# huangeddie/GymGo

Hardware: AMD Instinct MI355X
Metric: env steps/sec across batched games, 19x19 uniform-random rollouts (higher is better)
Workload: dtype u8; 1 GPU; 19x19, 65536 parallel games, uniform-random rollouts with auto-reset; one bench step = one launch of 256 plies for every game; board=19, games=65536, games_per_gpu=65536, env_steps_per_bench_step=16777216, burn_in_steps=1, desync_plies=640

## Files before the change

### gymgo_amd/csrc/gg_r5.hip

```cpp
#include <hip/hip_runtime.h>
#include <stdint.h>

#include "gg_common.h"
#include "gg_v2.h"
#include "gg_v4.h"
#include "gg_v5.h"
#include "gg_ws.h"

namespace gg {

void launch_rollout5(int io, int N, uint8_t *st, uint64_t *rng, int32_t *last_actions, int64_t *steps_done, int64_t B, uint32_t inv,
                     int plies, int auto_reset, int nb, int grid, hipStream_t s, uint32_t *ws) {
#define GG_R5(R)                                                                                                                  \
  do {                                                                                                                            \
    if (io == 0) k_rollout5<R, 0><<<grid, kWave, 0, s>>>(st, rng, last_actions, steps_done, B, inv, plies, auto_reset, nb, ws);   \
    else k_rollout5<R, 2><<<grid, kWave, 0, s>>>(st, rng, last_actions, steps_done, B, inv, plies, auto_reset, nb, nullptr);      \
  } while (0)
  if (N == 19) GG_R5(19);
  else if (N == 13) GG_R5(13);
  else GG_R5(9);
#undef GG_R5
}

void launch_rollout5_policy(int N, uint8_t *st, uint64_t *rng, int32_t *last_actions, int64_t *steps_done, int64_t B, uint32_t inv,
                            int plies, int auto_reset, int nb, int grid, hipStream_t s) {
  if (N == 19) k_rollout5_pol<19, 2><<<grid, kWave, 0, s>>>(st, rng, last_actions, steps_done, B, inv, plies, auto_reset, nb, nullptr);
  else if (N == 13) k_rollout5_pol<13, 2><<<grid, kWave, 0, s>>>(st, rng, last_actions, steps_done, B, inv, plies, auto_reset, nb, nullptr);
  else k_rollout5_pol<9, 2><<<grid, kWave, 0, s>>>(st, rng, last_actions, steps_done, B, inv, plies, auto_reset, nb, nullptr);
}

}

#ifdef GG_AB_SWEEPS
extern "C" int32_t gg_ab_sweeps_read_r5(unsigned long long *out2) {
  if (hipDeviceSynchronize() != hipSuccess) return 1;
  if (hipMemcpyFromSymbol(out2, HIP_SYMBOL(gg::gg_sweeps), 16) != hipSuccess) return 2;
  unsigned long long z[2] = {0, 0};
  return hipMemcpyToSymbol(HIP_SYMBOL(gg::gg_sweeps), z, 16) == hipSuccess ? 0 : 3;
}
#endif

#ifdef GG_AB_PROF
GG_PROF_READ(gg_ab_prof_read_r5)
#endif

#ifdef GG_AB_P3
extern "C" int32_t gg_ab_p3_read_r5(unsigned long long *out10) {
  if (hipDeviceSynchronize() != hipSuccess) return 1;
  if (hipMemcpyFromSymbol(out10, HIP_SYMBOL(gg::gg_p3), 80) != hipSuccess) return 2;
  unsigned long long z[10] = {0, 0, 0, 0, 0, 0, 0, 0, 0, 0};
  return hipMemcpyToSymbol(HIP_SYMBOL(gg::gg_p3), z, 80) == hipSuccess ? 0 : 3;
}
#endif

#ifdef GG_AB_WS
extern "C" int32_t gg_ab_ws_read_r5(unsigned long long *out2) {
  if (hipDeviceSynchronize() != hipSuccess) return 1;
  if (hipMemcpyFromSymbol(out2, HIP_SYMBOL(gg::gg_wsc), 16) != hipSuccess) return 2;
  unsigned long long z[2] = {0, 0};
  return hipMemcpyToSymbol(HIP_SYMBOL(gg::gg_wsc), z, 16) == hipSuccess ? 0 : 3;
}
#endif

#ifdef GG_AB_LOADSPLIT
extern "C" int32_t gg_ab_load_split_read_r5(unsigned long long *out4) {
  if (hipDeviceSynchronize() != hipSuccess) return 1;
  if (hipMemcpyFromSymbol(out4, HIP_SYMBOL(gg::gg_lsplit), 32) != hipSuccess) return 2;
  unsigned long long z[4] = {0, 0, 0, 0};
  return hipMemcpyToSymbol(HIP_SYMBOL(gg::gg_lsplit), z, 32) == hipSuccess ? 0 : 3;
}
#endif

#if defined(GG_AB_P3) || defined(GG_AB_LIVE)
extern "C" int32_t gg_ab_live_bad_r5(unsigned long long *out1) {
  if (hipDeviceSynchronize() != hipSuccess) return 1;
  return hipMemcpyFromSymbol(out1, HIP_SYMBOL(gg::gg_live_bad), 8) == hipSuccess ? 0 : 2;
}
#endif
```

### gymgo_amd/csrc/gg_v5.h

```cpp
#pragma once
#include "gg_v4.h"

namespace gg {

constexpr int kNB5 = 32;
constexpr int kJobCap = 128;

template <int R>
struct Lds5 {
  static constexpr int RS = R == 13 ? 20 : Cfg<R>::kRowStride;
  static constexpr int RPL = (R + 1) / 2;
  static_assert(2 * RPL <= RS, "a pair's rows must fit the row stride");
  static constexpr int kPad = 4;
  static constexpr int kState = kPad;
  static constexpr int kMeta = kState + 2 * kNB5 * RS;
  static constexpr int kFair = kMeta + 5 * kNB5;
  static constexpr int kTmp = kFair + 16;
  static constexpr int kUnion = kTmp + 4 * RS;
  static constexpr int kZero = kJobCap, kDump = kJobCap + 1;
  static constexpr int kCls = kUnion;
  static constexpr int kJob = kCls + kJobCap + 4;
  static constexpr int kG = kJob + kJobCap + 4;
  static constexpr int kSc = kG + 2 * kNB5 * RS;
  static constexpr int kLoopEnd = kSc + kWave * RS;
  static constexpr int kV2 = kUnion;
  static constexpr int kIoEnd = kV2 + (Lds2<R>::kRegion0 > 768 ? Lds2<R>::kRegion0 : 768);
  static constexpr int kDmaWords = (((kNB5 * (5 * R + 1) * 4 + 12 + 15) / 16 + kWave - 1) / kWave) * 256;
  static constexpr int kDmaEnd = kUnion + kDmaWords;
  static constexpr int kGrpBits = kUnion;
  static constexpr int kGrpWords = ((15 + kNB5 * 6 * R * R + 31) / 32 + 4) & ~3;
  static constexpr int kGrpLut = kGrpBits + kGrpWords;
  static constexpr int kGrpEnd = kGrpLut + 512;
  static constexpr int kMax2(int a, int b) { return a > b ? a : b; }
  static constexpr int kTotal = kMax2(kMax2(kLoopEnd, kIoEnd), kMax2(kDmaEnd, kGrpEnd));
  static_assert(kTotal * 4 <= 20480, "two waves per SIMD: 20 KB of LDS per wave");
  static_assert(kUnion % 4 == 0 && kG % 4 == 0 && kSc % 4 == 0, "16-byte alignment of the flood blocks");
  static_assert(3 * kNB5 * RS <= kLoopEnd - kUnion, "parked tracked rows fit the loop area");
};

__device__ __forceinline__ uint32_t mbcnt64(uint64_t m) {
  return __builtin_amdgcn_mbcnt_hi((uint32_t)(m >> 32), __builtin_amdgcn_mbcnt_lo((uint32_t)m, 0u));
}
constexpr int QP_L0 = 0xA0;

__device__ __forceinline__ void kth_set_bit10(const uint32_t (&v)[10], const uint32_t (&p)[10], uint32_t tt, int &rr, uint32_t &pos) {
  uint32_t ntt = ~tt;
  const uint32_t g5 = (uint32_t)((int32_t)(p[4] + ntt) >> 31);
  uint32_t a[5], t[4];
#pragma unroll
  for (int i = 0; i < 5; ++i) a[i] = B3(g5, v[5 + i], v[i], T_SEL);
#pragma unroll
  for (int i = 0; i < 4; ++i) t[i] = B3(g5, p[5 + i], p[i], T_SEL);
  uint32_t base = g5 & p[4], row = g5 & 5u;
  const uint32_t g2 = (uint32_t)((int32_t)(t[1] + ntt) >> 31);
  const uint32_t b0 = B3(g2, a[2], a[0], T_SEL), b1 = B3(g2, a[3], a[1], T_SEL), u0 = B3(g2, t[2], t[0], T_SEL);
  base = B3(g2, t[1], base, T_SEL);
  row = B3(g2, 2u, row, T_ANDOR);
  const uint32_t g1 = (uint32_t)((int32_t)(u0 + ntt) >> 31);
  uint32_t vr = B3(g1, b1, b0, T_SEL);
  base = B3(g1, u0, base, T_SEL);
  row -= g1;
  const uint32_t g1b = B3(g2, g1, (uint32_t)((int32_t)(t[3] + ntt) >> 31), TA & TB & TC);
  vr = B3(g1b, a[4], vr, T_SEL);
  base = B3(g1b, t[3], base, T_SEL);
  row -= g1b;
  ntt += base;
  uint32_t ps = 0;
#pragma unroll
  for (int sh = 16; sh >= 1; sh >>= 1) {
    const uint32_t e = (uint32_t)__popc((vr >> ps) & ((1u << sh) - 1u)) + ntt;
    const uint32_t ge = (uint32_t)((int32_t)e >> 31);
    ntt = B3(ge, e, ntt, T_SEL);
    ps = B3((uint32_t)sh, ge, ps, T_ANDOR);
  }
  rr = (int)row;
  pos = ps;
}

template <int R, bool WEAK>
__device__ __forceinline__ void flood_jobs(const uint32_t (&m)[R], const uint32_t (&mrev)[R], uint32_t (&f)[R], uint32_t (&res)[R],
                                           bool need, const uint32_t (&mm)[R], uint32_t &open) {
  int sweeps = 0;
#pragma unroll 1
  for (int it = 0; it < R * R; ++it) {
#pragma unroll
    for (int r = 0; r < R; ++r) FLOOD_VISIT(r, r - 1, (r & 1) != 0);
    if (it > 0) {
      uint32_t op = 0, opw = 0, pend = 0, above = 0;
#pragma unroll
      for (int r = R - 1; r >= 0; --r) {
        const uint32_t g = ((r + 1) & 1) ? __brev(f[r]) : f[r];
        res[r] = g;
        if (r < R - 1) {
          const uint32_t t = B3(above, m[r], g, T_AND_ANDN);
          if (WEAK) { op |= t; opw = B3(t, mm[r], opw, (TA & ~TB & 0xFF) | TC); }
          else or_pairs(op, pend, (R - 2 - r) & 1, t);
        }
        above = g;
      }
      if (!WEAK && ((R - 1) & 1)) op |= pend;
      open = op;
      if (__ballot((WEAK ? opw : op) != 0 && need) == 0) { sweeps = 2 * it + 1; break; }
    }
#pragma unroll
    for (int r = R - 1; r >= 0; --r) FLOOD_VISIT(r, r + 1, ((r + 1) & 1) != 0);
    if (it > 0) {
      uint32_t op = 0, opw = 0, pend = 0, below = 0;
#pragma unroll
      for (int r = 0; r < R; ++r) {
        const uint32_t g = (r & 1) ? __brev(f[r]) : f[r];
        res[r] = g;
        if (r > 0) {
          const uint32_t t = B3(below, m[r], g, T_AND_ANDN);
          if (WEAK) { op |= t; opw = B3(t, mm[r], opw, (TA & ~TB & 0xFF) | TC); }
          else or_pairs(op, pend, (r - 1) & 1, t);
        }
        below = g;
      }
      if (!WEAK && ((R - 1) & 1)) op |= pend;
      open = op;
      if (__ballot((WEAK ? opw : op) != 0 && need) == 0) { sweeps = 2 * it + 2; break; }
    }
  }
#ifdef GG_AB_SWEEPS
  { int l_; asm volatile("v_mbcnt_lo_u32_b32 %0, -1, 0\n\tv_mbcnt_hi_u32_b32 %0, -1, %0" : "=v"(l_));
    if (l_ == 0) { atomicAdd(&gg_sweeps[0], (unsigned long long)sweeps); atomicAdd(&gg_sweeps[1], 1ull); } }
#endif
  (void)sweeps;
}

template <int R>
__device__ __forceinline__ uint32_t job_liberties(const uint32_t (&gt)[R], const uint32_t (&ot)[R], const uint32_t (&m)[R]) {
  constexpr uint32_t FULLROW = (1u << R) - 1u;
  uint32_t o3[3] = {0u, 0u, 0u}, d3[3] = {0u, 0u, 0u};
#pragma unroll
  for (int r = 0; r < R; ++r) {
    const uint32_t e = B3(ot[r], m[r], FULLROW, ~(TA | TB) & TC & 0xFF);
    const uint32_t up = r > 0 ? gt[r - 1] : 0u, dn = r + 1 < R ? gt[r + 1] : 0u;
    const uint32_t dd = B3(shl1(gt[r]), gt[r] >> 1, up, T_OR3);
    const uint32_t l = B3(dd, dn, e, (TA | TB) & TC);
    d3[r % 3] = B3(l, o3[r % 3], d3[r % 3], T_ANDOR);
    o3[r % 3] = B3(l, o3[r % 3], 0u, T_OR3);
  }
  const uint32_t o = B3(o3[0], o3[1], o3[2], T_OR3);
  const uint32_t d = B3(d3[0], d3[1], d3[2], T_OR3) | B3(o3[0], o3[1], o3[2], T_MAJ);
  const uint32_t two = B3(o - 1u, o, d, T_ANDOR);
  return (o != 0u ? 1u : 0u) + (two != 0u ? 1u : 0u);
}

#ifdef GG_AB_P3
static __device__ unsigned long long gg_p3[10];
#define GG_P3(k, n) (p3c_[k] += (n))
#else
#define GG_P3(k, n) ((void)0)
#endif
#ifdef GG_AB_MARK
#define GG_MARK(k) asm volatile("; GGMARK " #k ::: "memory")
#else
#define GG_MARK(k) do {} while (0)
#endif
#if defined(GG_AB_P3) || defined(GG_AB_LIVE)
#define GG_LIVE_CHECK 1
static __device__ unsigned long long gg_live_bad;
#endif

#ifdef GG_AB_WS
static __device__ unsigned long long gg_wsc[2];
#define GG_WSC_DECL uint32_t wsc_[2] = {0u, 0u}
#define GG_WSC(hit) (wsc_[(hit) ? 0 : 1] += 1u)
#define GG_WSC_FLUSH do { if (ws && ln0 == 0) { atomicAdd(&gg_wsc[0], (unsigned long long)wsc_[0]); \
    atomicAdd(&gg_wsc[1], (unsigned long long)wsc_[1]); } } while (0)
#else
#define GG_WSC_DECL do {} while (0)
#define GG_WSC(hit) ((void)0)
#define GG_WSC_FLUSH do {} while (0)
#endif
#ifdef GG_AB_LOADSPLIT
static __device__ unsigned long long gg_lsplit[4];
#define GG_LS_DECL unsigned long long tls_[3] = {0, 0, 0}, tlc_ = clock64()
#define GG_LS(k) do { asm volatile("s_waitcnt lgkmcnt(0)" ::: "memory"); __builtin_amdgcn_sched_barrier(0); \
    const unsigned long long n_ = clock64(); __builtin_amdgcn_sched_barrier(0); tls_[k] += n_ - tlc_; tlc_ = n_; } while (0)
#define GG_LS_START do { __builtin_amdgcn_sched_barrier(0); tlc_ = clock64(); __builtin_amdgcn_sched_barrier(0); } while (0)
#define GG_LS_FLUSH do { if (ln0 == 0) { for (int k_ = 0; k_ < 3; ++k_) atomicAdd(&gg_lsplit[k_], tls_[k_]); \
    atomicAdd(&gg_lsplit[3], 1ull); } } while (0)
#else
#define GG_LS_DECL do {} while (0)
#define GG_LS(k) do {} while (0)
#define GG_LS_START do {} while (0)
#define GG_LS_FLUSH do {} while (0)
#endif

#define GG_R5_NAME k_rollout5
#define GG_R5_POL kPolUniform
#include "gg_v5_kernel.h"
#undef GG_R5_NAME
#undef GG_R5_POL
#define GG_R5_NAME k_rollout5_pol
#define GG_R5_POL kPolNoEyeFill
#include "gg_v5_kernel.h"
#undef GG_R5_NAME
#undef GG_R5_POL

}
```

### gymgo_amd/csrc/gg_v5_kernel.h

```cpp
template <int R, int IO>
__global__ __launch_bounds__(kWave, 2) void GG_R5_NAME(uint8_t *__restrict__ states, uint64_t *__restrict__ rng,
                                                       int32_t *__restrict__ last_actions, int64_t *__restrict__ steps_done,
                                                       int64_t B, uint32_t inv, int plies, int auto_reset, int nb,
                                                       uint32_t *__restrict__ ws) {
  constexpr int POL = GG_R5_POL;
  static_assert(IO == 0 || IO == 2, "byte planes or tracked boards");
  constexpr int N = R;
  constexpr int RS = Lds5<R>::RS;
  constexpr int RV = (R + 3) / 4;
  constexpr int RPL = Lds5<R>::RPL;
  constexpr int PL = kNB5 * RS;
  constexpr int ZERO = Lds5<R>::kZero, DUMP = Lds5<R>::kDump;
  constexpr bool TRACKED = IO == 2;
  constexpr int P = N * N, S = 6 * P, W = 5 * N + 1;
  constexpr uint32_t FULLROW = (1u << N) - 1u;
  __shared__ __attribute__((aligned(16))) uint32_t lds[Lds5<R>::kTotal];
  uint32_t *st = lds + Lds5<R>::kState;
  uint32_t *flagsv = lds + Lds5<R>::kMeta;
  int *lastv = reinterpret_cast<int *>(lds + Lds5<R>::kMeta + kNB5);
  int *playedv = reinterpret_cast<int *>(lds + Lds5<R>::kMeta + 2 * kNB5);
  uint32_t *rngv = lds + Lds5<R>::kMeta + 3 * kNB5;
  uint32_t *tmp = lds + Lds5<R>::kTmp;
  uint32_t *clsv = lds + Lds5<R>::kCls;
  uint32_t *jobv = lds + Lds5<R>::kJob;
  uint32_t *gblk = lds + Lds5<R>::kG;
  uint32_t *sc = lds + Lds5<R>::kSc;
  uint32_t *v2 = lds + Lds5<R>::kV2;
  uint32_t *park = lds + Lds5<R>::kUnion;
  const int64_t ngroups = (B + nb - 1) / nb;

  for (int64_t g = blockIdx.x; g < ngroups; g += gridDim.x) {
    const int64_t b_first = g * nb;
    int ln0;
    asm volatile("v_mbcnt_lo_u32_b32 %0, -1, 0\n\tv_mbcnt_hi_u32_b32 %0, -1, %0" : "=v"(ln0));
    const Half hf = make_half(ln0, N, inv);
    const bool row = hf.hl < RS;
    const int s5 = hf.lane >> 1, t2 = hf.lane & 1, r05 = RPL * t2;
    uint32_t inv_r[RPL], M[RPL];
#pragma unroll
    for (int r = 0; r < RPL; ++r) inv_r[r] = M[r] = 0u;
    uint32_t wsmiss = 0;
    GG_WSC_DECL;
    GG_LS_DECL;
    GG_PROF_DECL;
    WAVE_SYNC();
    if (TRACKED) {
      const int64_t nbrd = (B - b_first) < nb ? (B - b_first) : nb;
      const int nw = (int)nbrd * W;
      const uint32_t *gp = reinterpret_cast<const uint32_t *>(states) + b_first * (int64_t)W;
      constexpr int KD = Lds5<R>::kDmaWords / 256;
      const uint8_t *gb = reinterpret_cast<const uint8_t *>(gp);
      const uint32_t mis = (uint32_t)((uintptr_t)gb & 15u);
      const int nvec = (int)((mis + (uint32_t)nw * 4u + 15u) >> 4);
      WAVE_SYNC();
      lds_drain();
      {
        const uint32_t stage_lds = lds_addr(park);
#pragma unroll
        for (int k = 0; k < KD; ++k) {
          const int v = hf.lane + kWave * k;
          if (v < nvec) dma16(gb - mis + 16 * v, stage_lds + 1024u * (uint32_t)k);
        }
      }
      uint64_t xg = 0;
      if (hf.lane < kNB5) xg = rng[(hf.lane < nb && b_first + hf.lane < B) ? b_first + hf.lane : B - 1];
      for (int i = hf.lane; i < 2 * PL; i += kWave) st[i] = 0;
      if (hf.lane < Lds5<R>::kPad) lds[hf.lane] = 0;
      dma_wait();
      WAVE_SYNC();
      const uint32_t *stg = reinterpret_cast<const uint32_t *>(reinterpret_cast<const uint8_t *>(park) + mis);
      for (int i = hf.lane; i < (int)nbrd * 2 * N; i += kWave) {
        const int sb = i / (2 * N), w = i - sb * (2 * N);
        const int pl = w >= N ? 1 : 0;
        st[pl * PL + sb * RS + (w - pl * N)] = stg[sb * W + w];
      }
      if (hf.lane < kNB5) {
        const int sb = hf.lane;
        const bool on = sb < nb && b_first + sb < B;
        flagsv[sb] = on ? ((stg[sb * W + 5 * N] & 7u) | 8u) : 0u;
        lastv[sb] = -1;
        playedv[sb] = 0;
        rngv[2 * sb] = (uint32_t)xg;
        rngv[2 * sb + 1] = (uint32_t)(xg >> 32);
      }
      {
        const bool have = s5 < (int)nbrd;
        const uint32_t *bq = stg + (have ? s5 : 0) * W;
#pragma unroll
        for (int r = 0; r < RPL; ++r) {
          const int rw = r05 + r;
          const bool ok = have && rw < N;
          const int rc = ok ? rw : 0;
          const uint32_t iv = bq[2 * N + rc], mb = bq[3 * N + rc], mw = bq[4 * N + rc];
          inv_r[r] = ok ? iv : 0u;
          M[r] = ok ? (mb | mw) : 0u;
        }
      }
      WAVE_SYNC();
    } else {
      if (hf.lane < kNB5) flagsv[hf.lane] = 0;
      for (int i = hf.lane; i < 2 * PL; i += kWave) st[i] = 0;
      if (hf.lane < Lds5<R>::kPad) lds[hf.lane] = 0;
      WAVE_SYNC();
      constexpr int NVL = (4 * R * R + 15 + 15) / 512 + 1;
      static_assert(NVL <= 3, "vectors per lane of a staged board");
      if (hf.lane < kNB5) {
        const uint64_t x = rng[(b_first + hf.lane < B) ? b_first + hf.lane : B - 1];
        rngv[2 * hf.lane] = (uint32_t)x;
        rngv[2 * hf.lane + 1] = (uint32_t)(x >> 32);
      }
      uint4 cv0 = make_uint4(0, 0, 0, 0), cv1 = cv0, cv2 = cv0, nv0 = cv0, nv1 = cv0, nv2 = cv0;
      uint32_t cfb = 0, nfb = 0;
      uint32_t cw0 = 0, cw1 = 0, cw2 = 0, cw3 = 0, nw0 = 0, nw1 = 0, nw2 = 0, nw3 = 0;
#define GG_ISSUE_WS5(I, A0, A1, A2, A3)                                                                                \
      do {                                                                                                             \
        const int s_ = 2 * (I) + hf.h;                                                                                 \
        const int64_t b_ = (b_first + s_ < B) ? b_first + s_ : B - 1;                                                  \
        if (hf.hl < N) {                                                                                               \
          const uint32_t *wp_ = ws + b_ * (int64_t)W + hf.hl;                                                          \
          A0 = wp_[0]; A1 = wp_[N]; A2 = wp_[3 * N]; A3 = wp_[4 * N];                                                  \
        }                                                                                                              \
      } while (0)
#define GG_ISSUE_PAIR5(I, V0, V1, V2, FB)                                                                              \
      do {                                                                                                             \
        const int s_ = 2 * (I) + hf.h;                                                                                 \
        const int64_t b_ = (b_first + s_ < B) ? b_first + s_ : B - 1;                                                  \
        const uint8_t *gs_ = states + b_ * (int64_t)S;                                                                 \
        FB = 0;                                                                                                        \
        if (hf.hl < 4) {                                                                                               \
          const int off_ = hf.hl == 0 ? 2 * P : hf.hl == 1 ? 3 * P : hf.hl == 2 ? 4 * P : 5 * P;                       \
          FB = gs_[off_];                                                                                              \
        }                                                                                                              \
        const uint32_t mis_ = (uint32_t)((uintptr_t)gs_ & 15u);                                                        \
        const uint4 *ga_ = reinterpret_cast<const uint4 *>(gs_ - mis_);                                                \
        const int nv_ = (int)(mis_ + 4 * P + 15) >> 4;                                                                 \
        if (hf.hl < nv_) V0 = ga_[hf.hl];                                                                              \
        if (NVL > 1 && hf.hl + 32 < nv_) V1 = ga_[hf.hl + 32];                                                         \
        if (NVL > 2 && hf.hl + 64 < nv_) V2 = ga_[hf.hl + 64];                                                         \
      } while (0)
      if (nb >= 2) GG_ISSUE_PAIR5(0, cv0, cv1, cv2, cfb);
      if (ws && nb >= 2) GG_ISSUE_WS5(0, cw0, cw1, cw2, cw3);
#pragma unroll 1
      for (int i = 0; i < nb / 2; ++i) {
        if (i + 1 < nb / 2) GG_ISSUE_PAIR5(i + 1, nv0, nv1, nv2, nfb);
        if (ws && i + 1 < nb / 2) GG_ISSUE_WS5(i + 1, nw0, nw1, nw2, nw3);
        const int s = 2 * i + hf.h;
        const bool on = b_first + s < B;
        const int64_t b = on ? b_first + s : B - 1;
        uint32_t black, white, invalid, mb = 0, mw = 0;
        const uint8_t *gs = states + b * (int64_t)S;
        uint8_t *io = reinterpret_cast<uint8_t *>(v2) + hf.h * Cfg<R>::kIoBytes;
        const uint32_t mi = (uint32_t)((uintptr_t)gs & 15u);
        const int nv = (int)(mi + 4 * P + 15) >> 4;
        GG_LS_START;
        const uint32_t flags = half_of(__ballot(cfb != 0), hf.h) & 0xFu;
        WAVE_SYNC();
        uint4 *iov = reinterpret_cast<uint4 *>(io);
        if (hf.hl < nv) iov[hf.hl] = cv0;
        if (NVL > 1 && hf.hl + 32 < nv) iov[hf.hl + 32] = cv1;
        if (NVL > 2 && hf.hl + 64 < nv) iov[hf.hl + 64] = cv2;
        WAVE_SYNC();
        black = plane_to_row<R>(io + mi, N, hf.hl);
        white = plane_to_row<R>(io + mi + P, N, hf.hl);
        invalid = plane_to_row<R>(io + mi + 3 * P, N, hf.hl);
        const uint32_t turn = flags & 1u, passed = (flags >> 2) & 1u, done = (flags >> 3) & 1u;
        GG_LS(0);
        bool known = false;
        if (ws) {
          known = __ballot(hf.hl < N && (black != cw0 || white != cw1)) == 0;
          if (known) { mb = cw2; mw = cw3; }
          else wsmiss |= 3u << (2 * i);
          GG_WSC(known);
        }
        if (!known) {
          uint32_t ab;
          analyze2<R, false>(black, white, hf.full_l1 & ~(black | white), hf, v2, mb, ab, mw, nullptr, nullptr, true);
        }
        GG_LS(1);
        if (row) {
          st[0 * PL + s * RS + hf.hl] = black;
          st[1 * PL + s * RS + hf.hl] = white;
          tmp[(hf.h * 2 + 0) * RS + hf.hl] = invalid;
          tmp[(hf.h * 2 + 1) * RS + hf.hl] = mb | mw;
        }
        if (hf.hl == 0) {
          flagsv[s] = turn | (passed << 1) | (done << 2) | (on ? 8u : 0u);
          lastv[s] = -1;
          playedv[s] = 0;
        }
        WAVE_SYNC();
        if ((hf.lane >> 2) == i) {
          const uint32_t *tp = tmp + ((s5 & 1) * 2) * RS + r05;
#pragma unroll
          for (int r = 0; r < RPL; ++r) {
            inv_r[r] = tp[r];
            M[r] = tp[RS + r];
          }
        }
        WAVE_SYNC();
        GG_LS(2);
        cv0 = nv0; cv1 = nv1; cv2 = nv2; cfb = nfb;
        if (ws) { cw0 = nw0; cw1 = nw1; cw2 = nw2; cw3 = nw3; }
      }
#undef GG_ISSUE_PAIR5
#undef GG_ISSUE_WS5
      GG_LS_FLUSH;
    }
    WAVE_SYNC();
    for (int i = hf.lane; i < kWave * RS; i += kWave) sc[i] = 0u;
    WAVE_SYNC();

    uint32_t flr = flagsv[s5];
    const uint64_t x0r = ((uint64_t)rngv[2 * s5 + 1] << 32) | rngv[2 * s5];
    int playedr = 0;
#ifdef GG_AB_P3
    uint32_t p3c_[10] = {0, 0, 0, 0, 0, 0, 0, 0, 0, 0};
#endif
#ifdef GG_LIVE_CHECK
    int drawsr = 0;
    bool was_dead = false;
#endif
    GG_PROF(6);
    FairShare fair(lds + Lds5<R>::kFair);
    const uint32_t fair_lag = plies >= 192 ? 24u : (plies >= 16 ? (uint32_t)plies >> 3 : 2u);
    bool lead = false;
    uint32_t uq = 0;
#pragma unroll 1
    for (int t = 0; t < plies; ++t) {
      if ((t & 3) == 0 && plies >= 8) {
        const uint32_t left = (uint32_t)(plies - t);
        lead = fair.behind((uint32_t)t, left < fair_lag ? (left > 2u ? left : 2u) : fair_lag) != 0u;
        if (lead) __builtin_amdgcn_s_setprio(2); else __builtin_amdgcn_s_setprio(3);
      }
      int ln;
      asm volatile("v_mbcnt_lo_u32_b32 %0, -1, 0\n\tv_mbcnt_hi_u32_b32 %0, -1, %0" : "=v"(ln));
      const int s4 = (ln >> 1) & 31, t5 = ln & 1, r0 = RPL * t5;
      const bool bl = s4 < nb;
      uint32_t full[RPL];
#pragma unroll
      for (int r = 0; r < RPL; ++r) full[r] = (r0 + r < N) ? FULLROW : 0u;

      int a_q;
      uint32_t fl_q;
      {
        const uint32_t fl = flr;
        const bool on = bl && ((fl >> 3) & 1u);
        const bool done = (fl >> 2) & 1u;
        const bool live = on && !(done && !auto_reset);
        const bool reset = live && done;
#ifdef GG_LIVE_CHECK
        if (live && was_dead) atomicAdd(&gg_live_bad, 1ull);
        was_dead = was_dead || (bl && !live);
        drawsr += live ? 1 : 0;
#endif
        uint32_t v[RPL], p[RPL];
        const uint32_t rm = reset ? ~0u : 0u;
        uint32_t eye[RPL];
        if constexpr (POL == kPolNoEyeFill) {
          const uint32_t turn = fl & 1u;
          const uint32_t *pm = st + turn * PL + s4 * RS + r0, *po = st + (1u - turn) * PL + s4 * RS + r0;
          uint32_t me[RPL], op[RPL];
#pragma unroll
          for (int r = 0; r < RPL; ++r) { me[r] = pm[r]; op[r] = po[r]; }
          const uint32_t me_up = dpp0<QP_X1>(me[RPL - 1]), op_up = dpp0<QP_X1>(op[RPL - 1]);
          const uint32_t me_dn = dpp0<QP_X1>(me[0]), op_dn = dpp0<QP_X1>(op[0]);
#pragma unroll
          for (int r = 0; r < RPL; ++r) {
            const int rw = r0 + r;
            const uint32_t meU = r ? me[r - 1] : (t5 ? me_up : FULLROW), opU = r ? op[r - 1] : (t5 ? op_up : 0u);
            const uint32_t meDn = r + 1 < RPL ? me[r + 1] : (t5 ? 0u : me_dn), opD = r + 1 < RPL ? op[r + 1] : (t5 ? 0u : op_dn);
            const uint32_t meD = rw + 1 >= N ? FULLROW : meDn;
            const uint32_t edge = (rw == 0 || rw == N - 1) ? FULLROW : (1u | (1u << (N - 1)));
            eye[r] = eye_row(me[r], op[r], meU, meD, opU, opD, full[r], edge, N) & ~rm;
          }
        }
#pragma unroll
        for (int r = 0; r < RPL; ++r) {
          v[r] = B3(full[r], rm, inv_r[r], TA & (TB | (~TC & 0xFF)));
          if constexpr (POL == kPolNoEyeFill) v[r] &= ~eye[r];
          p[r] = (uint32_t)__popc(v[r]) + (r ? p[r - 1] : 0u);
        }
        const uint32_t T = p[RPL - 1];
        const uint32_t oth = dpp0<QP_X1>(T);
        const uint32_t Pb = t5 ? oth : 0u, n = T + oth;
        if ((t & 1) == 0) {
          uint64_t xx = x0r + (uint64_t)(uint32_t)(t + t5) * 0x9E3779B97F4A7C15ull;
          uq = (uint32_t)(splitmix_next(xx) >> 32);
        }
        const uint32_t uh = dpp0<QP_L0>(uq);
        uq = dpp0<QP_X1>(uq);
        const uint32_t k = __umulhi(uh, POL == kPolNoEyeFill ? n : n + 1u);
        const bool hit = k >= Pb && k < Pb + T;
        int rr;
        uint32_t pos;
        if constexpr (RPL == 10) kth_set_bit10(v, p, (k - Pb) & 0x3FFu, rr, pos);
        else kth_set_bit<RPL>(v, p, (k - Pb) & 0x3FFu, rr, pos);
        const int rabs = r0 + rr;
        const uint32_t cand = hit ? (uint32_t)(rabs * N + (int)pos) : 0u;
        const uint32_t pt = cand | dpp0<QP_X1>(cand);
        a_q = !live ? -1 : (k < n ? (int)pt : P);
        const bool place = live && hit;
        fl_q = reset ? 40u : fl;
        uint64_t resetm = __ballot(reset && t5 == 0);
        const bool none_live = __ballot(live) == 0;
        if (none_live && resetm == 0) break;
        if (resetm) {
          if (reset) {
#pragma unroll
            for (int r = 0; r < RPL; ++r) inv_r[r] = M[r] = 0u;
          }
          while (resetm) {
            const int s = (__ffsll((unsigned long long)resetm) - 1) >> 1;
            resetm &= resetm - 1;
            for (int i = hf.lane; i < 2 * RS; i += kWave) st[(i / RS) * PL + s * RS + (i % RS)] = 0;
            if (hf.lane == 0) flagsv[s] = 8u | 32u;
          }
          if (none_live) break;
        }
        WAVE_SYNC();
        uint32_t *gb = gblk + 2 * s4 * RS;
        if (t5 == 0) clsv[s4] = 0u;
        {
          uint4 *pz = reinterpret_cast<uint4 *>(gb + t5 * RS);
#pragma unroll
          for (int i = 0; i < RV; ++i) pz[i] = make_uint4(0u, 0u, 0u, 0u);
        }
        asm volatile("" ::: "memory");
        if (place) {
          const int turn = reset ? 0 : (int)(fl & 1u);
          atomicOr(st + turn * PL + s4 * RS + rabs, 1u << pos);
          gb[rabs] = 1u << pos;
        }
      }
      WAVE_SYNC();
      GG_PROF(0);

      uint32_t qs;
      int njobs;
      {
        const int a = a_q;
        const uint32_t turn = fl_q & 1u;
        const uint32_t mv1 = ((uint32_t)a < (uint32_t)P) ? 1u : 0u;
        int ar, ac;
        split_action(mv1 ? a : 0, N, inv, ar, ac);
        const uint32_t *pm = st + turn * PL + s4 * RS, *po = st + (1u - turn) * PL + s4 * RS;
        uint32_t obit[2], packed = 0;
#pragma unroll
        for (int j = 0; j < 2; ++j) {
          const int sg = 2 * j - 1;
          const int dr = t5 ? 0 : sg, dc = t5 ? sg : 0;
          const int nr = ar + dr, nc = ac + dc;
          const uint32_t rowm = pm[nr], rowo = po[nr];
          const uint32_t ncs = (uint32_t)nc & 31u;
          const uint32_t mbit = (rowm >> ncs) & mv1, ob = (rowo >> ncs) & mv1;
          const uint32_t onb = ((uint32_t)nr < (uint32_t)N && (uint32_t)nc < (uint32_t)N) ? mv1 : 0u;
          const uint32_t ex = mbit | ob;
          packed += (onb & ~ex) | (mbit << 8) | ((onb & ~ob) << 16);
          obit[j] = ob;
        }
        qs = packed + dpp0<QP_X1>(packed) + 0x70700u;
        const uint32_t friendly = (qs >> 11) & 1u;
        const uint32_t gf = t5 ? 0u : friendly;
        const uint32_t c = gf + obit[0] + obit[1];
        const uint64_t b0 = __ballot((c & 1u) != 0u), b1 = __ballot((c & 2u) != 0u);
        const uint32_t base = mbcnt64(b0) + 2u * mbcnt64(b1);
        njobs = (int)__popcll(b0) + 2 * (int)__popcll(b1);
        const uint32_t sG = base, s0 = base + gf, s1 = s0 + obit[0];
        const uint32_t common = (uint32_t)s4 | (1u << 18) | ((turn ^ 1u) << 15);
        const int step = t5 ? 1 : N;
        jobv[gf ? sG : (uint32_t)DUMP] = ((uint32_t)s4 | (1u << 18) | (turn << 15) | (1u << 16)) | ((uint32_t)a << 5);
        const uint32_t dirs = (uint32_t)t5 << 20;
        jobv[obit[0] ? s0 : (uint32_t)DUMP] = common | dirs | ((uint32_t)(a - step) << 5);
        jobv[obit[1] ? s1 : (uint32_t)DUMP] = common | dirs | (1u << 19) | ((uint32_t)(a + step) << 5);
      }
      WAVE_SYNC();

      if (plies >= 8) { if (lead) __builtin_amdgcn_s_setprio(0); else __builtin_amdgcn_s_setprio(1); }
#pragma unroll 1
      for (int jb = 0; jb < njobs; jb += kWave) {
        const int j = jb + ln;
        const bool have = j < njobs;
        const uint32_t d = jobv[have ? j : DUMP];
        const uint32_t ex = have ? 1u : 0u;
        const int sj = (int)(d & 31u);
        int sr, scol;
        split_action((int)((d >> 5) & 511u), N, inv, sr, scol);
        const uint32_t ownc = (d >> 15) & 1u;
        const uint32_t isG = have ? (d >> 16) & 1u : 0u;
        uint32_t *blk = sc + ln * RS;
        const uint4 *lds4 = reinterpret_cast<const uint4 *>(lds);
        const uint4 *pmv = lds4 + (Lds5<R>::kState + (int)ownc * PL + sj * RS) / 4;
        const uint4 *pov = lds4 + (Lds5<R>::kState + (int)(ownc ^ 1u) * PL + sj * RS) / 4;
        uint32_t mm[R];
        {
          const int src = 8 * sj;
#pragma unroll
          for (int i = 0; i < RPL; ++i) {
            mm[i] = (uint32_t)__builtin_amdgcn_ds_bpermute(src, (int)M[i]);
            if (RPL + i < R) mm[RPL + i] = (uint32_t)__builtin_amdgcn_ds_bpermute(src + 4, (int)M[i]);
          }
        }
        uint32_t cnt = 0;
        uint32_t res[R];
        {
          uint32_t m[R], mrev[R], f[R], ot[R];
          {
            uint32_t mt[RV * 4], ft[RV * 4];
#pragma unroll
            for (int i = 0; i < RV; ++i) {
              const uint4 x = pmv[i], y = pov[i];
              mt[4 * i] = x.x; mt[4 * i + 1] = x.y; mt[4 * i + 2] = x.z; mt[4 * i + 3] = x.w;
              ot[4 * i] = y.x;
              if (4 * i + 1 < R) ot[4 * i + 1] = y.y;
              if (4 * i + 2 < R) ot[4 * i + 2] = y.z;
              if (4 * i + 3 < R) ot[4 * i + 3] = y.w;
            }
            {
              const int srw = sr & (int)(0u - ex);
              asm volatile("" ::: "memory");
              blk[srw] = ex << (((uint32_t)scol ^ (0u - ((uint32_t)sr & 1u))) & 31u);
              asm volatile("" ::: "memory");
              const uint4 *pf = reinterpret_cast<const uint4 *>(blk);
#pragma unroll
              for (int i = 0; i < RV; ++i) {
                const uint4 x = pf[i];
                ft[4 * i] = x.x; ft[4 * i + 1] = x.y; ft[4 * i + 2] = x.z; ft[4 * i + 3] = x.w;
              }
              asm volatile("" ::: "memory");
              blk[srw] = 0u;
            }
#pragma unroll
            for (int r = 0; r < R; ++r) {
              m[r] = mt[r];
              mrev[r] = __brev(m[r]);
              f[r] = ft[r];
              res[r] = 0u;
            }
          }
          GG_PROF(1);
          uint32_t open = 0;
          flood_jobs<R, true>(m, mrev, f, res, isG != 0u, mm, open);
          GG_PROF(2);
          cnt = job_liberties<R>(res, ot, m);
          const bool unsettled = have && open != 0u && cnt < 2u;
          if (__ballot(unsettled)) {
#pragma unroll
            for (int r = 0; r < R; ++r) f[r] = (r & 1) ? __brev(res[r]) : res[r];
            flood_jobs<R, false>(m, mrev, f, res, unsettled, mm, open);
            cnt = job_liberties<R>(res, ot, m);
          }
        }
        const uint32_t lib2 = cnt < 2u ? cnt : 2u;
        uint32_t *gb = gblk + 2 * sj * RS;
        if (isG) {
          uint4 *pz = reinterpret_cast<uint4 *>(gb);
#pragma unroll
          for (int i = 0; i < RV; ++i)
            pz[i] = make_uint4(res[4 * i], 4 * i + 1 < R ? res[4 * i + 1] : 0u, 4 * i + 2 < R ? res[4 * i + 2] : 0u, 4 * i + 3 < R ? res[4 * i + 3] : 0u);
          if (lib2) atomicOr(clsv + sj, lib2 << 4);
        } else if (have && cnt < 2u) {
          static_assert(Lds5<R>::kG % 2 == 0 && RS % 2 == 0 && R + 1 <= RS, "8-byte aligned row pairs inside the block");
#pragma unroll
          for (int r = 0; r < R; r += 2) {
            const uint32_t hi = r + 1 < R ? res[r + 1] : 0u;
            atomicOr(reinterpret_cast<unsigned long long *>(gb + RS + r), ((unsigned long long)hi << 32) | res[r]);
          }
          if (cnt == 0u) atomicOr(clsv + sj, 1u << ((d >> 19) & 3u));
        }
      }
      if (plies >= 8) { if (lead) __builtin_amdgcn_s_setprio(2); else __builtin_amdgcn_s_setprio(3); }
      WAVE_SYNC();
      GG_PROF(3);

      {
        const int a = a_q;
        const uint32_t fl = fl_q;
        const uint32_t info = clsv[s4];
        const int turn0 = fl & 1u;
        uint32_t *pmine = st + turn0 * PL + s4 * RS + r0;
        uint32_t *popp = st + (1 - turn0) * PL + s4 * RS + r0;
        const uint32_t *gG = gblk + 2 * s4 * RS + r0;
        uint32_t mine1[RPL], opp0[RPL], all4[RPL], bg[RPL];
#pragma unroll
        for (int r = 0; r < RPL; ++r) {
          mine1[r] = pmine[r];
          opp0[r] = popp[r];
          bg[r] = gG[r];
          all4[r] = gG[RS + r];
        }
        const bool moves_now = a >= 0;
        const bool is_pass = a == P;
        int ar, ac;
        split_action(a, N, inv, ar, ac);
        const uint32_t capt_m = info & 15u;
        uint32_t g0[RPL], opp1[RPL];
#pragma unroll
        for (int r = 0; r < RPL; ++r) {
          g0[r] = bg[r];
          opp1[r] = B3(opp0[r], all4[r], M[r], TA & ~(TB & ~TC) & 0xFF);
        }
        const uint32_t ne = qs & 7u, ne2 = ne < 2u ? ne : 2u;
        uint32_t libsG = ((qs >> 11) & 1u) ? ((info >> 4) & 3u) : ne2;
        uint32_t ko_oh = 0, ko_bit = 0;
        GG_P3(0, 1u);
        GG_P3(8, (uint32_t)__popcll(__ballot(capt_m != 0u && t5 == 0)));
        GG_P3(9, (uint32_t)__popcll(__ballot(a >= 0 && t5 == 0)));
        GG_MARK(10);
        if (__ballot(capt_m != 0u)) {
          GG_MARK(11);
          GG_P3(1, 1u);
          uint32_t cap[RPL];
#pragma unroll
          for (int r = 0; r < RPL; ++r) cap[r] = B3(all4[r], M[r], M[r], TA & ~TB & 0xFF);
          const uint32_t ncapn = (uint32_t)__popc(capt_m);
          if (__ballot(ncapn == 1u && libsG == 0u)) {
            GG_MARK(12);
            GG_P3(2, 1u);
            uint32_t dg[RPL];
            dilate_rows<RPL>(g0, dg);
            uint32_t cntc = 0;
#pragma unroll
            for (int r = 0; r < RPL; ++r) cntc += (uint32_t)__popc(dg[r] & cap[r]);
            const uint32_t c2 = cntc < 2u ? cntc : 2u;
            const uint32_t tot = c2 + dpp0<QP_X1>(c2);
            libsG += (ncapn == 1u && libsG == 0u) ? (tot < 2u ? tot : 2u) : ncapn;
            GG_MARK(13);
          } else {
            libsG += ncapn;
          }
          const bool ko1 = ncapn == 1u && !(qs & CL_OPEN);
          if (__ballot(ko1)) {
            GG_MARK(14);
            GG_P3(3, 1u);
            uint32_t died = 0;
#pragma unroll
            for (int r = 0; r < RPL; ++r) died += (uint32_t)__popc(cap[r]);
            const bool ko = ko1 && died + dpp0<QP_X1>(died) == 1u;
            const uint32_t kr = (uint32_t)ar - (capt_m & 1u) + ((capt_m >> 1) & 1u) - (uint32_t)r0;
            ko_oh = (ko && kr < (uint32_t)RPL) ? (1u << (kr & 31)) : 0u;
            ko_bit = 1u << (((uint32_t)ac - ((capt_m >> 2) & 1u) + (capt_m >> 3)) & 31u);
            GG_MARK(15);
          }
          GG_MARK(16);
          uint32_t atari[RPL], f[RPL], anyf = 0;
          {
            const uint32_t up = dpp0<0x138>(cap[RPL - 1]), dn = dpp0<0x130>(cap[0]);
#pragma unroll
            for (int r = 0; r < RPL; ++r) {
              atari[r] = B3(mine1[r], M[r], g0[r], TA & ~(TB | TC) & 0xFF);
              const uint32_t above = r == 0 ? up : cap[r - 1], below = r == RPL - 1 ? dn : cap[r + 1];
              const uint32_t v = B3(cap[r] >> 1, above, below, T_OR3);
              f[r] = B3(shl1(cap[r]), v, atari[r], (TA | TB) & TC);
              anyf |= f[r];
            }
          }
          GG_MARK(17);
          if (__ballot(anyf != 0u)) {
            GG_MARK(18);
            GG_P3(5, 1u);
#ifdef GG_AB_P3
            uint32_t trips_ = 0;
#define GG_TRIP ++trips_
#else
#define GG_TRIP do {} while (0)
#endif
#define GG_JOIN_TRIP(R0, D)                                                                                               \
            do {                                                                                                          \
              GG_TRIP;                                                                                                    \
              const uint32_t up_ = dpp0<0x138>(f[RPL - 1]), dn_ = dpp0<0x130>(f[0]);                                      \
              chg = 0;                                                                                                    \
              _Pragma("unroll") for (int i_ = 0; i_ < RPL; ++i_) {                                                        \
                const int r_ = (R0) + (D) * i_;                                                                           \
                const uint32_t above_ = r_ == 0 ? up_ : f[r_ == 0 ? 0 : r_ - 1];                                          \
                const uint32_t below_ = r_ == RPL - 1 ? dn_ : f[r_ == RPL - 1 ? 0 : r_ + 1];                              \
                const uint32_t v_ = B3(f[r_] >> 1, above_, below_, T_OR3);                                              \
                const uint32_t g_ = B3(shl1(f[r_]), v_, atari[r_], (TA | TB) & TC);                                      \
                chg = B3(g_, f[r_], chg, (TA & ~TB & 0xFF) | TC);                                                         \
                f[r_] |= g_;                                                                                              \
              }                                                                                                           \
            } while (0)
            uint32_t chg;
#pragma unroll 1
            for (int it = 0; it < R * R; ++it) {
              GG_JOIN_TRIP(0, 1);
              if (__ballot(chg != 0u) == 0) break;
              GG_JOIN_TRIP(RPL - 1, -1);
              if (__ballot(chg != 0u) == 0) break;
            }
#undef GG_JOIN_TRIP
#undef GG_TRIP
#ifdef GG_AB_P3
            GG_P3(6, trips_);
            p3c_[7] = trips_ > p3c_[7] ? trips_ : p3c_[7];
#endif
#pragma unroll
            for (int r = 0; r < RPL; ++r) M[r] |= f[r];
            GG_MARK(19);
          }
        }
        GG_MARK(20);
        const uint32_t gsel = libsG >= 2u ? ~0u : 0u;
        uint32_t e[RPL], x[RPL], nbr[RPL];
#pragma unroll
        for (int r = 0; r < RPL; ++r) {
          const uint32_t u = B3(M[r], g0[r], all4[r], TA & ~(TB | TC) & 0xFF);
          M[r] = B3(gsel, g0[r], u, T_ANDOR);
          const uint32_t y = B3(M[r], mine1[r], opp1[r], T_SEL);
          x[r] = B3(full[r], y, y, TA & ~TB & 0xFF);
          e[r] = B3(full[r], opp1[r], mine1[r], TA & ~(TB | TC) & 0xFF);
        }
        dilate_rows<RPL>(x, nbr);
        const uint32_t mv_m = moves_now ? ~0u : 0u;
#pragma unroll
        for (int r = 0; r < RPL; ++r) {
          const uint32_t invalid = B3(e[r], nbr[r], full[r], ~(TA & TB) & TC & 0xFF);
          inv_r[r] = B3(mv_m, invalid, inv_r[r], T_SEL);
        }
        if (__ballot(ko_oh != 0u)) {
#pragma unroll
          for (int r = 0; r < RPL; ++r) inv_r[r] |= (uint32_t)__builtin_amdgcn_sbfe((int)ko_oh, r, 1) & ko_bit;
        }
        if (capt_m) {
#pragma unroll
          for (int r = 0; r < RPL; ++r) popp[r] = opp1[r];
        }
        flr = fl;
        if (moves_now) {
          const uint32_t passed0 = (fl >> 1) & 1u, done0 = (fl >> 2) & 1u;
          const uint32_t passed = is_pass ? 1u : 0u, done = done0 | (passed & passed0);
          flr = (uint32_t)(turn0 ^ 1) | (passed << 1) | (done << 2) | 8u | (fl & 32u);
          playedr += 1;
          if (t5 == 0) {
            flagsv[s4] = flr;
            lastv[s4] = a;
            playedv[s4] = playedr;
          }
        }
      }
      WAVE_SYNC();
      GG_PROF(4);
    }
    if (plies >= 8) fair.release();
    GG_PROF(5);
#ifdef GG_AB_P3
    if (ln0 == 0) {
#pragma unroll
      for (int k = 0; k < 10; ++k) {
        if (k == 7) atomicMax(&gg_p3[7], (unsigned long long)p3c_[7]);
        else atomicAdd(&gg_p3[k], (unsigned long long)p3c_[k]);
      }
    }
#endif
#ifdef GG_LIVE_CHECK
    if (playedr != drawsr) atomicAdd(&gg_live_bad, 1ull);
#endif

    int lnS;
    asm volatile("v_mbcnt_lo_u32_b32 %0, -1, 0\n\tv_mbcnt_hi_u32_b32 %0, -1, %0" : "=v"(lnS));
    const int s5s = lnS >> 1, r05s = RPL * (lnS & 1);
    WAVE_SYNC();
    if (TRACKED) {
#pragma unroll
      for (int r = 0; r < RPL; ++r) {
        if (r05s + r < RS) {
          const uint32_t bk = st[0 * PL + s5s * RS + r05s + r], wh = st[1 * PL + s5s * RS + r05s + r];
          park[0 * PL + s5s * RS + r05s + r] = inv_r[r];
          park[1 * PL + s5s * RS + r05s + r] = M[r] & bk;
          park[2 * PL + s5s * RS + r05s + r] = M[r] & wh;
        }
      }
      WAVE_SYNC();
      const int64_t nbrd = (B - b_first) < nb ? (B - b_first) : nb;
      const int nw = (int)nbrd * W;
      uint32_t *gp = reinterpret_cast<uint32_t *>(states) + b_first * (int64_t)W;
      bool tch = false;
      if (lnS < (int)nbrd) tch = playedv[lnS] != 0 || (flagsv[lnS] & 32u);
      const uint64_t tmask = __ballot(tch);
#pragma unroll 1
      for (int i0 = lnS; i0 < nw; i0 += 4 * kWave) {
        uint32_t v[4];
        bool ok[4];
#pragma unroll
        for (int k = 0; k < 4; ++k) {
          const int i = i0 + k * kWave;
          const int ic = i < nw ? i : 0;
          const int sb = ic / W, w = ic - sb * W;
          ok[k] = i < nw && ((tmask >> sb) & 1ull);
          const int pl = w / N, rw = w - pl * N;
          const uint32_t *src = pl >= 5 ? flagsv + sb : (pl < 2 ? st + pl * PL + sb * RS + rw : park + (pl - 2) * PL + sb * RS + rw);
          const uint32_t x = *src;
          v[k] = pl >= 5 ? (x & 7u) : x;
        }
#pragma unroll
        for (int k = 0; k < 4; ++k)
          if (ok[k]) gp[i0 + k * kWave] = v[k];
      }
      if (lnS < nb && b_first + lnS < B) {
        const int sb = lnS;
        const int64_t b = b_first + sb;
        const int played = playedv[sb];
        rng[b] = (((uint64_t)rngv[2 * sb + 1] << 32) | rngv[2 * sb]) + (uint64_t)(uint32_t)played * 0x9E3779B97F4A7C15ull;
        if (last_actions) last_actions[b] = lastv[sb];
        if (steps_done && played) atomicAdd(reinterpret_cast<unsigned long long *>(steps_done) + b, (unsigned long long)played);
      }
      WAVE_SYNC();
    } else {
      const int nbrd = (int)((B - b_first) < nb ? (B - b_first) : nb);
      bool any_wr = false;
      if (lnS < nbrd) any_wr = playedv[lnS] != 0 || (flagsv[lnS] & 32u);
      if (__ballot(any_wr))
        emit_group<R, RPL, 2>(states + b_first * (int64_t)S, nbrd, N, st, PL, RS, inv_r, flagsv, lds + Lds5<R>::kGrpBits,
                              reinterpret_cast<uint2 *>(lds + Lds5<R>::kGrpLut), lnS);
      if (lnS < nbrd) {
        const int sb = lnS;
        const int64_t b = b_first + sb;
        const int played = playedv[sb];
        rng[b] = (((uint64_t)rngv[2 * sb + 1] << 32) | rngv[2 * sb]) + (uint64_t)(uint32_t)played * 0x9E3779B97F4A7C15ull;
        if (last_actions) last_actions[b] = lastv[sb];
        if (steps_done && played) atomicAdd(reinterpret_cast<unsigned long long *>(steps_done) + b, (unsigned long long)played);
      }
      WAVE_SYNC();
      if (ws) {
        const uint64_t wmask = __ballot(lnS < nbrd && (any_wr || ((wsmiss >> (lnS & 31)) & 1u)));
        if (wmask) {
#pragma unroll
          for (int r = 0; r < RPL; ++r) {
            if (r05s + r < RS) {
              const uint32_t bk = st[0 * PL + s5s * RS + r05s + r], wh = st[1 * PL + s5s * RS + r05s + r];
              park[0 * PL + s5s * RS + r05s + r] = M[r] & bk;
              park[1 * PL + s5s * RS + r05s + r] = M[r] & wh;
            }
          }
          WAVE_SYNC();
          uint32_t *wg = ws + b_first * (int64_t)W;
          const int nw4 = nbrd * 4 * N;
#pragma unroll 1
          for (int i0 = lnS; i0 < nw4; i0 += 4 * kWave) {
            uint32_t v[4];
            int at[4];
#pragma unroll
            for (int k = 0; k < 4; ++k) {
              const int i = i0 + k * kWave;
              const int ic = i < nw4 ? i : 0;
              const int sb = ic / (4 * N), w = ic - sb * (4 * N);
              const int pl = w / N, rw = w - pl * N;
              v[k] = pl < 2 ? st[pl * PL + sb * RS + rw] : park[(pl - 2) * PL + sb * RS + rw];
              at[k] = (i < nw4 && ((wmask >> sb) & 1ull)) ? sb * W + (pl < 2 ? w : w + N) : -1;
            }
#pragma unroll
            for (int k = 0; k < 4; ++k)
              if (at[k] >= 0) wg[at[k]] = v[k];
          }
          WAVE_SYNC();
        }
      }
    }
    GG_WSC_FLUSH;
    GG_PROF(7);
    GG_PROF_FLUSH;
  }
}
```

Before: 13.87 billion env steps/s.

## Merge two-phase flood into one resumable loop with earlier closure test on 19x19

```diff
diff --git a/gymgo_amd/csrc/gg_r5.hip b/gymgo_amd/csrc/gg_r5.hip
--- a/gymgo_amd/csrc/gg_r5.hip
+++ b/gymgo_amd/csrc/gg_r5.hip
@@ -32,11 +32,11 @@
 }
 
 #ifdef GG_AB_SWEEPS
-extern "C" int32_t gg_ab_sweeps_read_r5(unsigned long long *out2) {
+extern "C" int32_t gg_ab_sweeps_read_r5(unsigned long long *out10) {
   if (hipDeviceSynchronize() != hipSuccess) return 1;
-  if (hipMemcpyFromSymbol(out2, HIP_SYMBOL(gg::gg_sweeps), 16) != hipSuccess) return 2;
-  unsigned long long z[2] = {0, 0};
-  return hipMemcpyToSymbol(HIP_SYMBOL(gg::gg_sweeps), z, 16) == hipSuccess ? 0 : 3;
+  if (hipMemcpyFromSymbol(out10, HIP_SYMBOL(gg::gg_sweeps5), 80) != hipSuccess) return 2;
+  unsigned long long z[10] = {0, 0, 0, 0, 0, 0, 0, 0, 0, 0};
+  return hipMemcpyToSymbol(HIP_SYMBOL(gg::gg_sweeps5), z, 80) == hipSuccess ? 0 : 3;
 }
 #endif
 
diff --git a/gymgo_amd/csrc/gg_v5.h b/gymgo_amd/csrc/gg_v5.h
--- a/gymgo_amd/csrc/gg_v5.h
+++ b/gymgo_amd/csrc/gg_v5.h
@@ -77,57 +77,18 @@
   pos = ps;
 }
 
-template <int R, bool WEAK>
-__device__ __forceinline__ void flood_jobs(const uint32_t (&m)[R], const uint32_t (&mrev)[R], uint32_t (&f)[R], uint32_t (&res)[R],
-                                           bool need, const uint32_t (&mm)[R], uint32_t &open) {
-  int sweeps = 0;
-#pragma unroll 1
-  for (int it = 0; it < R * R; ++it) {
-#pragma unroll
-    for (int r = 0; r < R; ++r) FLOOD_VISIT(r, r - 1, (r & 1) != 0);
-    if (it > 0) {
-      uint32_t op = 0, opw = 0, pend = 0, above = 0;
-#pragma unroll
-      for (int r = R - 1; r >= 0; --r) {
-        const uint32_t g = ((r + 1) & 1) ? __brev(f[r]) : f[r];
-        res[r] = g;
-        if (r < R - 1) {
-          const uint32_t t = B3(above, m[r], g, T_AND_ANDN);
-          if (WEAK) { op |= t; opw = B3(t, mm[r], opw, (TA & ~TB & 0xFF) | TC); }
-          else or_pairs(op, pend, (R - 2 - r) & 1, t);
-        }
-        above = g;
-      }
-      if (!WEAK && ((R - 1) & 1)) op |= pend;
-      open = op;
-      if (__ballot((WEAK ? opw : op) != 0 && need) == 0) { sweeps = 2 * it + 1; break; }
-    }
-#pragma unroll
-    for (int r = R - 1; r >= 0; --r) FLOOD_VISIT(r, r + 1, ((r + 1) & 1) != 0);
-    if (it > 0) {
-      uint32_t op = 0, opw = 0, pend = 0, below = 0;
-#pragma unroll
-      for (int r = 0; r < R; ++r) {
-        const uint32_t g = (r & 1) ? __brev(f[r]) : f[r];
-        res[r] = g;
-        if (r > 0) {
-          const uint32_t t = B3(below, m[r], g, T_AND_ANDN);
-          if (WEAK) { op |= t; opw = B3(t, mm[r], opw, (TA & ~TB & 0xFF) | TC); }
-          else or_pairs(op, pend, (r - 1) & 1, t);
-        }
-        below = g;
-      }
-      if (!WEAK && ((R - 1) & 1)) op |= pend;
-      open = op;
-      if (__ballot((WEAK ? opw : op) != 0 && need) == 0) { sweeps = 2 * it + 2; break; }
-    }
-  }
-#ifdef GG_AB_SWEEPS
-  { int l_; asm volatile("v_mbcnt_lo_u32_b32 %0, -1, 0\n\tv_mbcnt_hi_u32_b32 %0, -1, %0" : "=v"(l_));
-    if (l_ == 0) { atomicAdd(&gg_sweeps[0], (unsigned long long)sweeps); atomicAdd(&gg_sweeps[1], 1ull); } }
-#endif
-  (void)sweeps;
-}
+template <int R>
+constexpr int flood_first_test() {
+#ifdef GG_AB_FLOODK
+  return R == 19 ? GG_AB_FLOODK : 3;
+#else
+  return R == 19 ? 2 : 3;
+#endif
+}
+
+#ifdef GG_AB_SWEEPS
+static __device__ unsigned long long gg_sweeps5[10];
+#endif
 
 template <int R>
 __device__ __forceinline__ uint32_t job_liberties(const uint32_t (&gt)[R], const uint32_t (&ot)[R], const uint32_t (&m)[R]) {
@@ -146,6 +107,132 @@
   const uint32_t d = B3(d3[0], d3[1], d3[2], T_OR3) | B3(o3[0], o3[1], o3[2], T_MAJ);
   const uint32_t two = B3(o - 1u, o, d, T_ANDOR);
   return (o != 0u ? 1u : 0u) + (two != 0u ? 1u : 0u);
+}
+
+template <int R, bool WEAK>
+__device__ __forceinline__ void flood_jobs_restart(const uint32_t (&m)[R], const uint32_t (&mrev)[R], uint32_t (&f)[R], uint32_t (&res)[R],
+                                           bool need, const uint32_t (&mm)[R], uint32_t &open) {
+  int sweeps = 0;
+#pragma unroll 1
+  for (int it = 0; it < R * R; ++it) {
+#pragma unroll
+    for (int r = 0; r < R; ++r) FLOOD_VISIT(r, r - 1, (r & 1) != 0);
+    if (it > 0) {
+      uint32_t op = 0, opw = 0, pend = 0, above = 0;
+#pragma unroll
+      for (int r = R - 1; r >= 0; --r) {
+        const uint32_t g = ((r + 1) & 1) ? __brev(f[r]) : f[r];
+        res[r] = g;
+        if (r < R - 1) {
+          const uint32_t t = B3(above, m[r], g, T_AND_ANDN);
+          if (WEAK) { op |= t; opw = B3(t, mm[r], opw, (TA & ~TB & 0xFF) | TC); }
+          else or_pairs(op, pend, (R - 2 - r) & 1, t);
+        }
+        above = g;
+      }
+      if (!WEAK && ((R - 1) & 1)) op |= pend;
+      open = op;
+      if (__ballot((WEAK ? opw : op) != 0 && need) == 0) { sweeps = 2 * it + 1; break; }
+    }
+#pragma unroll
+    for (int r = R - 1; r >= 0; --r) FLOOD_VISIT(r, r + 1, ((r + 1) & 1) != 0);
+    if (it > 0) {
+      uint32_t op = 0, opw = 0, pend = 0, below = 0;
+#pragma unroll
+      for (int r = 0; r < R; ++r) {
+        const uint32_t g = (r & 1) ? __brev(f[r]) : f[r];
+        res[r] = g;
+        if (r > 0) {
+          const uint32_t t = B3(below, m[r], g, T_AND_ANDN);
+          if (WEAK) { op |= t; opw = B3(t, mm[r], opw, (TA & ~TB & 0xFF) | TC); }
+          else or_pairs(op, pend, (r - 1) & 1, t);
+        }
+        below = g;
+      }
+      if (!WEAK && ((R - 1) & 1)) op |= pend;
+      open = op;
+      if (__ballot((WEAK ? opw : op) != 0 && need) == 0) { sweeps = 2 * it + 2; break; }
+    }
+  }
+  (void)sweeps;
+}
+
+template <int R>
+__device__ __forceinline__ uint32_t flood_jobs(const uint32_t (&m)[R], const uint32_t (&mrev)[R], uint32_t (&f)[R], uint32_t (&res)[R],
+                                               const uint32_t (&ot)[R], const uint32_t (&mm)[R], bool isG, bool have) {
+  constexpr int K = flood_first_test<R>();
+  static_assert(K >= 1 && K <= 3, "the first closure test comes after one, two or three sweeps");
+  uint32_t cnt = 0;
+  bool resumed = false;
+#ifdef GG_AB_SWEEPS
+  int sw_ = 0, sw0_ = 0;
+  uint32_t ng_ = 0, no_ = 0;
+#define GG_SW5_SWEEP() (++sw_)
+#else
+#define GG_SW5_SWEEP() ((void)0)
+#endif
+  auto done = [&](uint32_t op, uint32_t opw) -> bool {
+    if (!resumed && __ballot(opw != 0u && isG) != 0) return false;
+    cnt = job_liberties<R>(res, ot, m);
+    const bool unsettled = have && op != 0u && cnt < 2u;
+    const uint64_t u = __ballot(unsettled);
+#ifdef GG_AB_SWEEPS
+    if (!resumed) { sw0_ = sw_; ng_ = (uint32_t)__popcll(__ballot(unsettled && isG)); no_ = (uint32_t)__popcll(u) - ng_; }
+#endif
+    resumed = true;
+    return u == 0;
+  };
+#pragma unroll 1
+  for (int it = 0; it < R * R; ++it) {
+#pragma unroll
+    for (int r = 0; r < R; ++r) FLOOD_VISIT(r, r - 1, (r & 1) != 0);
+    GG_SW5_SWEEP();
+    if (K <= 1 || it > 0) {
+      uint32_t op = 0, opw = 0, above = 0;
+#pragma unroll
+      for (int r = R - 1; r >= 0; --r) {
+        const uint32_t g = ((r + 1) & 1) ? __brev(f[r]) : f[r];
+        res[r] = g;
+        if (r < R - 1) {
+          const uint32_t t = B3(above, m[r], g, T_AND_ANDN);
+          op |= t;
+          opw = B3(t, mm[r], opw, (TA & ~TB & 0xFF) | TC);
+        }
+        above = g;
+      }
+      if (done(op, opw)) break;
+    }
+#pragma unroll
+    for (int r = R - 1; r >= 0; --r) FLOOD_VISIT(r, r + 1, ((r + 1) & 1) != 0);
+    GG_SW5_SWEEP();
+    if (K <= 2 || it > 0) {
+      uint32_t op = 0, opw = 0, below = 0;
+#pragma unroll
+      for (int r = 0; r < R; ++r) {
+        const uint32_t g = (r & 1) ? __brev(f[r]) : f[r];
+        res[r] = g;
+        if (r > 0) {
+          const uint32_t t = B3(below, m[r], g, T_AND_ANDN);
+          op |= t;
+          opw = B3(t, mm[r], opw, (TA & ~TB & 0xFF) | TC);
+        }
+        below = g;
+      }
+      if (done(op, opw)) break;
+    }
+  }
+#undef GG_SW5_SWEEP
+#ifdef GG_AB_SWEEPS
+  { int l_; asm volatile("v_mbcnt_lo_u32_b32 %0, -1, 0\n\tv_mbcnt_hi_u32_b32 %0, -1, %0" : "=v"(l_));
+    if (l_ == 0) {
+      const int ex_ = sw_ - sw0_;
+      atomicAdd(&gg_sweeps5[0], (unsigned long long)sw0_); atomicAdd(&gg_sweeps5[1], 1ull);
+      if (ng_ + no_) { atomicAdd(&gg_sweeps5[2], 1ull); atomicAdd(&gg_sweeps5[2 + (ex_ < 4 ? ex_ : 4)], 1ull); }
+      atomicAdd(&gg_sweeps5[7], (unsigned long long)ng_); atomicAdd(&gg_sweeps5[8], (unsigned long long)no_);
+      atomicAdd(&gg_sweeps5[9], (unsigned long long)ex_);
+    } }
+#endif
+  return cnt;
 }
 
 #ifdef GG_AB_P3
diff --git a/gymgo_amd/csrc/gg_v5_kernel.h b/gymgo_amd/csrc/gg_v5_kernel.h
--- a/gymgo_amd/csrc/gg_v5_kernel.h
+++ b/gymgo_amd/csrc/gg_v5_kernel.h
@@ -438,16 +438,21 @@
             }
           }
           GG_PROF(1);
-          uint32_t open = 0;
-          flood_jobs<R, true>(m, mrev, f, res, isG != 0u, mm, open);
-          GG_PROF(2);
-          cnt = job_liberties<R>(res, ot, m);
-          const bool unsettled = have && open != 0u && cnt < 2u;
-          if (__ballot(unsettled)) {
-#pragma unroll
-            for (int r = 0; r < R; ++r) f[r] = (r & 1) ? __brev(res[r]) : res[r];
-            flood_jobs<R, false>(m, mrev, f, res, unsettled, mm, open);
+          if constexpr (R == 19) {
+            cnt = flood_jobs<R>(m, mrev, f, res, ot, mm, isG != 0u, have);
+            GG_PROF(2);
+          } else {
+            uint32_t open = 0;
+            flood_jobs_restart<R, true>(m, mrev, f, res, isG != 0u, mm, open);
+            GG_PROF(2);
             cnt = job_liberties<R>(res, ot, m);
+            const bool unsettled = have && open != 0u && cnt < 2u;
+            if (__ballot(unsettled)) {
+#pragma unroll
+              for (int r = 0; r < R; ++r) f[r] = (r & 1) ? __brev(res[r]) : res[r];
+              flood_jobs_restart<R, false>(m, mrev, f, res, unsettled, mm, open);
+              cnt = job_liberties<R>(res, ot, m);
+            }
           }
         }
         const uint32_t lib2 = cnt < 2u ? cnt : 2u;
```

Result: faster. 14.51 billion env steps/s, median of 6 (+4.7%).
